# Algy/fast-slic

Measured on AMD Instinct MI355X. Metric: megapixels/sec @10 iters (1280x720 & 4K, K=1600); % HBM roofline, higher is better.
Workload: dtype u8/u16/i32 (integer SLIC); 1 GPU; 1280x720 RGB, K=1600, 10 iters (configs[1]), 8 frames/GPU; frames_per_gpu=8, global_frames=8, slots_per_gpu=6, submissions_per_launch_group=up to 2 (dynamic batching of the pipeline), inputs=device-resident uint8 RGB, device int16 labels, parallelism=frames sharded across GPUs, no collective

## Files before the change

### fast_slic_amd/csrc/cca.hip

```cpp
#include "device_common.h"

namespace fslic {

constexpr uint32_t kNoAdopt = 0xFFFFFFFFu;
static __device__ __forceinline__ uint32_t* n_parent(const CcaDev& c, uint32_t n) { return reinterpret_cast<uint32_t*>(c.nrec + n); }
static __device__ __forceinline__ uint32_t n_leader(const CcaDev& c, uint32_t n) { return reinterpret_cast<const uint32_t*>(c.nrec + n)[1]; }
static __device__ __forceinline__ uint32_t n_local(const CcaDev& c, uint32_t n) { return reinterpret_cast<const uint32_t*>(c.nrec + n)[2]; }
static __device__ __forceinline__ uint32_t n_adopt(const CcaDev& c, uint32_t n) { return reinterpret_cast<const uint32_t*>(c.nrec + n)[3]; }

static __device__ __forceinline__ uint32_t lds_ld(uint32_t* p) {
    return __hip_atomic_load(p, __ATOMIC_RELAXED, __HIP_MEMORY_SCOPE_WORKGROUP);
}
static __device__ __forceinline__ void lds_st(uint32_t* p, uint32_t v) {
    __hip_atomic_store(p, v, __ATOMIC_RELAXED, __HIP_MEMORY_SCOPE_WORKGROUP);
}
static __device__ __forceinline__ uint32_t lds_find(uint32_t* par, uint32_t x) {
    for (;;) {
        const uint32_t p = lds_ld(par + x);
        if (p == x) return x;
        const uint32_t gp = lds_ld(par + p);
        if (gp == p) return p;
        lds_st(par + x, gp);
        x = gp;
    }
// ... 261 lines not shown
static __device__ __forceinline__ uint32_t g_load(uint32_t* p) {
    return __hip_atomic_load(p, __ATOMIC_RELAXED, __HIP_MEMORY_SCOPE_AGENT);
}
static __device__ __forceinline__ uint32_t node_at(const CcaDev& c, int y, int x, size_t p) {
    return (uint32_t)((y / kCcaTileH) * c.tiles_x + x / kCcaTile) * (uint32_t)kCcaTilePx + (uint32_t)c.lid[p];
}
static __device__ __forceinline__ uint32_t node_of(const CcaDev& c, uint32_t p) {
    const int y = (int)(p / (uint32_t)c.W);
    return node_at(c, y, (int)(p - (uint32_t)y * (uint32_t)c.W), p);
}
static __device__ __forceinline__ uint32_t g_find(const CcaDev& c, uint32_t x) {
    for (;;) {
        const uint32_t p = g_load(n_parent(c, x));
        if (p == x) return x;
        const uint32_t gp = g_load(n_parent(c, p));
        if (gp == p) return p;
        __hip_atomic_store(n_parent(c, x), gp, __ATOMIC_RELAXED, __HIP_MEMORY_SCOPE_AGENT);
        x = gp;
    }
}
static __device__ __forceinline__ void g_union(const CcaDev& c, uint32_t a, uint32_t b) {
    for (;;) {
        a = g_find(c, a);
        b = g_find(c, b);
        if (a == b) return;
        if (n_leader(c, a) < n_leader(c, b)) { const uint32_t t = a; a = b; b = t; }
        if (atomicCAS(n_parent(c, a), a, b) == a) return;
    }
}

static __device__ __forceinline__ uint2 g_load2(const CcaDev& c, uint32_t n) {
    const unsigned long long v = __hip_atomic_load(reinterpret_cast<unsigned long long*>(c.nrec + n), __ATOMIC_RELAXED, __HIP_MEMORY_SCOPE_AGENT);
    return make_uint2((uint32_t)v, (uint32_t)(v >> 32));
}
static __device__ __forceinline__ uint32_t g_find_leader(const CcaDev& c, uint32_t& x, uint2 r) {
    for (;;) {
        if (r.x == x) return r.y;
        const uint2 g = g_load2(c, r.x);
        if (g.x == r.x) { x = r.x; return g.y; }
        __hip_atomic_store(n_parent(c, x), g.x, __ATOMIC_RELAXED, __HIP_MEMORY_SCOPE_AGENT);
        x = g.x;
        r = g_load2(c, x);
    }
}
static __device__ __forceinline__ void g_union2(const CcaDev& c, uint32_t a, uint32_t b) {
    uint2 ra = g_load2(c, a), rb = g_load2(c, b);
    for (;;) {
        const uint32_t la = g_find_leader(c, a, ra), lb = g_find_leader(c, b, rb);
        if (a == b) return;
        if (la < lb) { const uint32_t t = a; a = b; b = t; }
        if (atomicCAS(n_parent(c, a), a, b) == a) return;
        ra = g_load2(c, a); rb = g_load2(c, b);
    }
}

#ifndef FSLIC_SEAM_PX
#define FSLIC_SEAM_PX 1
#endif
constexpr int kSeamPx = FSLIC_SEAM_PX;
__global__ __launch_bounds__(256) void k_cca_border(CcaDev c, int nh, int nv) {
    c.select(blockIdx.y);
    constexpr int T = kCcaTile;
    constexpr int TH = kCcaTileH;
    static_assert(TH % kSeamPx == 0 && T % kSeamPx == 0, "a thread's pixels lie in one tile");
    const int i = blockIdx.x * blockDim.x + threadIdx.x;
    const int W = c.W, H = c.H;
    if (i < nh) {
        const int cw = (W + kSeamPx - 1) / kSeamPx;
        const int sr = i / cw, x0 = (i - sr * cw) * kSeamPx;
        const int y = (sr + 1) * TH;
        const size_t p = (size_t)y * W + x0;
        uint32_t cur[kSeamPx + 1], up[kSeamPx + 1], nc[kSeamPx], nu[kSeamPx];
        const bool has_left = (x0 % T) != 0;
        cur[0] = has_left ? (uint32_t)c.in[p - 1] : 0x10000u;
        up[0] = has_left ? (uint32_t)c.in[p - W - 1] : 0x10000u;
#pragma unroll
        for (int q = 0; q < kSeamPx; ++q) {
            const bool ok = x0 + q < W;
            cur[q + 1] = ok ? (uint32_t)c.in[p + q] : 0x20000u;
            up[q + 1] = ok ? (uint32_t)c.in[p - W + q] : 0x30000u;
            nc[q] = ok ? (uint32_t)c.lid[p + q] : 0u;
            nu[q] = ok ? (uint32_t)c.lid[p - W + q] : 0u;
        }
        const uint32_t tile = (uint32_t)((sr + 1) * c.tiles_x + x0 / T) * (uint32_t)kCcaTilePx;
#pragma unroll
        for (int q = 0; q < kSeamPx; ++q) {
            const uint32_t lbl = cur[q + 1];
            if (up[q + 1] == lbl && (cur[q] != lbl || up[q] != lbl))
                g_union2(c, tile + nc[q], tile - (uint32_t)c.tiles_x * (uint32_t)kCcaTilePx + nu[q]);
        }
    } else if (i < nh + nv) {
        const int j = i - nh;
        const int ch = (H + kSeamPx - 1) / kSeamPx;
        const int bx = j / ch + 1, y0 = (j - (bx - 1) * ch) * kSeamPx;
        const int r0 = y0 % TH;
        const uint32_t tile_r = (uint32_t)((y0 / TH) * c.tiles_x + bx), tile_l = tile_r - 1u;
        const uint32_t* er = c.vedge + ((size_t)tile_r * TH + r0) * 2;
        const uint32_t* el = c.vedge + ((size_t)tile_l * TH + r0) * 2 + 1;
        uint32_t a[kSeamPx + 1], b[kSeamPx + 1];
        a[0] = r0 ? er[-2] : 0x10000u;
        b[0] = r0 ? el[-2] : 0x20000u;
#pragma unroll
        for (int q = 0; q < kSeamPx; ++q) {
            const bool ok = y0 + q < H;
            a[q + 1] = ok ? er[2 * q] : 0x10000u;
            b[q + 1] = ok ? el[2 * q] : 0x20000u;
        }
#pragma unroll
        for (int q = 0; q < kSeamPx; ++q) {
            const uint32_t lbl = a[q + 1] & 0xFFFFu;
            const bool contact = y0 + q < H && ((a[q + 1] ^ b[q + 1]) & 0xFFFFu) == 0u;
            const bool first = q + r0 == 0 || (a[q] & 0xFFFFu) != lbl || (b[q] & 0xFFFFu) != lbl;
            if (contact && first)
                g_union2(c, tile_r * (uint32_t)kCcaTilePx + (a[q + 1] >> 16), tile_l * (uint32_t)kCcaTilePx + (b[q + 1] >> 16));
        }
    }
}

__global__ __launch_bounds__(256) void k_cca_compress(CcaDev c, int nframes) {
    const uint32_t bx = blockIdx.x / (unsigned)nframes, nbx = gridDim.x / (unsigned)nframes;
    c.select((int)(blockIdx.x % (unsigned)nframes));
    const uint32_t r_first = c.roots[bx * blockDim.x + threadIdx.x];
    const uint32_t n = c.counters[0];
    const int lane = LANE();
    const uint32_t gstride = nbx * blockDim.x;
    const int64_t thr = (int64_t)c.min_threshold;
    __shared__ uint32_t s_app[2];
    for (uint32_t b0 = bx * blockDim.x; b0 < n; b0 += gstride) {
        const uint32_t i = b0 + threadIdx.x;
        if (threadIdx.x == 0) s_app[0] = 0u;
        __syncthreads();
        const bool live = i < n;
        const uint32_t r = (b0 == bx * blockDim.x && live) ? r_first : c.roots[min(i, n - 1)];
        const uint32_t a = n_local(c, r);
        uint32_t g = r;
        for (;;) {
            const uint32_t p = g_load(n_parent(c, g));
            if (p == g) break;
            g = p;
        }
        bool cand = false;
        if (live) {
            if (g == r) {
                c.nfinal[r] = 0xFFFFu;
                cand = (int64_t)a >= thr;
            } else {
                __hip_atomic_store(n_parent(c, r), g, __ATOMIC_RELAXED, __HIP_MEMORY_SCOPE_AGENT);
                const uint32_t old = atomicAdd(&c.narea[g], a);
                cand = (int64_t)old < thr && (int64_t)old + (int64_t)a >= thr;
            }
        }
        const int32_t leader = cand ? (int32_t)n_leader(c, g) : 0;
        const unsigned long long m = __ballot(cand);
        uint32_t wbase = 0;
        if (m && lane == 0) wbase = atomicAdd(&s_app[0], (uint32_t)__popcll(m));
        wbase = rfl(wbase);
        __syncthreads();
        if (threadIdx.x == 0 && s_app[0]) s_app[1] = atomicAdd(&c.counters[1], s_app[0]);
        __syncthreads();
        if (cand) {
            const uint32_t at = s_app[1] + wbase + (uint32_t)__popcll(m & ((1ull << lane) - 1ull));
            c.cand_leader[at] = leader;
            c.cand_area[at] = g;
        }
    }
}

constexpr int kSelCap = 10240;
constexpr int kSelSortCap = 8192;
constexpr int kSelBuckets = 2048;
constexpr int kSelBins = 4096;

static __device__ __forceinline__ uint32_t block_excl_scan_1024(uint32_t v, uint32_t* s_w, uint32_t& total) {
    const int lane = threadIdx.x & 63, wave = threadIdx.x >> 6;
    uint32_t inc = v;
#pragma unroll
    for (int off = 1; off < 64; off <<= 1) {
        const uint32_t u = __shfl_up(inc, off);
        if (lane >= off) inc += u;
    }
    __syncthreads();
    if (lane == 63) s_w[wave] = inc;
    __syncthreads();
    uint32_t base = 0, tot = 0;
#pragma unroll
    for (int w = 0; w < 16; ++w) {
        const uint32_t t = s_w[w];
        if (w < wave) base += t;
        tot += t;
    }
    total = tot;
    return base + inc - v;
}

static __device__ __forceinline__ void select_pass(const uint32_t* s_area, uint32_t M, int sh, bool first, uint32_t prefix,
                                                   uint32_t kk, uint32_t* s_hist, uint32_t* s_w, uint32_t* s_v) {
    const int tid = threadIdx.x;
    for (int i = tid; i < kSelBins; i += 1024) s_hist[i] = 0;
    __syncthreads();
    for (uint32_t i = tid; i < M; i += 1024) {
        const uint32_t a = s_area[i];
        if (first || (a >> (sh + 12)) == prefix) atomicAdd(&s_hist[(a >> sh) & (kSelBins - 1)], 1u);
    }
    __syncthreads();
    uint32_t h[4], tot = 0;
#pragma unroll
    for (int q = 0; q < 4; ++q) { h[q] = s_hist[kSelBins - 1 - 4 * tid - q]; tot += h[q]; }
    uint32_t total;
    uint32_t run = block_excl_scan_1024(tot, s_w, total);
#pragma unroll
    for (int q = 0; q < 4; ++q) {
        if (run < kk && run + h[q] >= kk) {
            s_v[1] = (uint32_t)(kSelBins - 1 - 4 * tid - q);
            s_v[2] = kk - run;
        }
        run += h[q];
    }
    __syncthreads();
}

typedef unsigned long long heap_t;
constexpr int kTieWaveLevels = 4;
static __device__ __forceinline__ heap_t hp_ld(heap_t* p) { return __hip_atomic_load(p, __ATOMIC_RELAXED, __HIP_MEMORY_SCOPE_WORKGROUP); }
static __device__ __forceinline__ void hp_st(heap_t* p, heap_t v) { __hip_atomic_store(p, v, __ATOMIC_RELAXED, __HIP_MEMORY_SCOPE_WORKGROUP); }
static __device__ __forceinline__ uint32_t hp_area(heap_t e) { return (uint32_t)(e >> 32); }

static __device__ __forceinline__ void tie_adjust_heap(heap_t* h, int hole, int len, heap_t value, bool writer, uint32_t astar) {
    const uint32_t vlim = min(hp_area(value), astar);
    int cur = hole;
    for (;;) {
        int child;
        heap_t em;
        if (cur < (len - 1) / 2) {
            child = 2 * (cur + 1);
            const heap_t e1 = hp_ld(h + child), e0 = hp_ld(h + child - 1);
            em = e1;
            if (hp_area(e1) > hp_area(e0)) { child--; em = e0; }
        } else if ((len & 1) == 0 && cur == (len - 2) / 2) {
            child = 2 * cur + 1;
            em = hp_ld(h + child);
        } else {
            break;
        }
        if (hp_area(em) > vlim) break;
        if (writer) hp_st(h + cur, em);
        cur = child;
    }
    if (writer) hp_st(h + cur, value);
}

static __device__ __forceinline__ uint32_t tie_wave_sift(heap_t* h, int len, int hole, heap_t value, int lane, uint32_t astar) {
    constexpr uint32_t kInf = 0xFFFFFFFFu;
    const uint32_t va = hp_area(value);
    const uint32_t vlim = min(va, astar);
    const int t = 31 - __clz(lane | 1);
    const int off = lane - (1 << t);
    int cur = hole;
    uint32_t at_hole = va;
    for (;;) {
        const long long idx = (((long long)(cur + 1)) << t) + off - 1;
        const bool ok = lane >= 1 && idx < (long long)len;
        const heap_t e = ok ? hp_ld(h + idx) : ((heap_t)kInf << 32);
        const uint32_t a = (uint32_t)(e >> 32);
        const uint32_t sib = (uint32_t)__builtin_amdgcn_update_dpp(0, (int)a, 0xB1 , 0xF, 0xF, true);
        const unsigned long long left_pref = __ballot(sib > a);
        const unsigned long long stop_at = __ballot(a > vlim);
        int c[5];
        uint32_t stops = 0;
        {
            int jj = 1;
#pragma unroll
            for (int s5 = 0; s5 < 5; ++s5) {
                const int cl = 2 * jj;
                c[s5] = cl + (int)(((left_pref >> cl) & 1ull) ^ 1ull);
                stops |= (uint32_t)((stop_at >> c[s5]) & 1ull) << s5;
                jj = c[s5];
            }
        }
        const int nmove = __builtin_ctz(stops | 32u);
        const bool stopped = nmove < 5;
        unsigned long long path = 0;
        int j = 1;
#pragma unroll
        for (int s5 = 0; s5 < 5; ++s5) {
            path |= s5 < nmove ? 1ull << c[s5] : 0ull;
            j = s5 < nmove ? c[s5] : j;
        }
        const long long pidx = (((long long)(cur + 1)) << max(t - 1, 0)) + (off >> 1) - 1;
        if ((path >> lane) & 1ull) hp_st(h + pidx, e);
        if (cur == hole && (path & 0xCull)) at_hole = (uint32_t)__builtin_amdgcn_readlane((int)a, (path & 4ull) ? 2 : 3);
        const int tj = 31 - __clz(j);
        cur = (int)((((long long)(cur + 1)) << tj) + (j - (1 << tj)) - 1);
        if (stopped || 2 * cur + 1 >= len) break;
    }
    if (lane == 0) hp_st(h + cur, value);
    return at_hole;
}

#if defined(FSLIC_LAB) && FSLIC_LAB == 1
#define SEL_STAMP(i_) do { if (threadIdx.x == 0) c.counters[4 + (i_)] = (uint32_t)__builtin_amdgcn_s_memrealtime(); } while (0)
#else
#define SEL_STAMP(i_) do { } while (0)
#endif
static __device__ __forceinline__ void tie_heap_select(const CcaDev& c, uint32_t M, uint32_t K, uint32_t astar, uint32_t* s_area, uint32_t* s_lead, uint32_t* s_key,
                                                       uint32_t* s_bcnt, uint32_t* s_bstart, uint32_t* s_bfill, uint32_t* s_w) {
    const int tid = threadIdx.x, lane = tid & 63;
    SEL_STAMP(2);
    constexpr int PER = kSelSortCap / 1024;
    int bsh = 0;
    while ((((uint32_t)c.N - 1u) >> bsh) >= (uint32_t)kSelBuckets) bsh++;
    for (int i = tid; i < 3 * kSelBuckets; i += 1024) s_bcnt[i] = 0;
    __syncthreads();
    for (uint32_t i = tid; i < M; i += 1024) atomicAdd(&s_bcnt[s_lead[i] >> bsh], 1u);
    __syncthreads();
    {
        const uint32_t a = s_bcnt[2 * tid], b = s_bcnt[2 * tid + 1];
        uint32_t tot;
        const uint32_t ex = block_excl_scan_1024(a + b, s_w, tot);
        s_bstart[2 * tid] = ex;
        s_bstart[2 * tid + 1] = ex + a;
    }
    __syncthreads();
    for (uint32_t i = tid; i < M; i += 1024) {
        const uint32_t b = s_lead[i] >> bsh;
        s_key[s_bstart[b] + atomicAdd(&s_bfill[b], 1u)] = s_lead[i];
    }
    __syncthreads();
    uint32_t my_lead[PER], my_area[PER], my_rank[PER];
#pragma unroll
    for (int q = 0; q < PER; ++q) {
        const uint32_t i = (uint32_t)tid + (uint32_t)q * 1024u;
        my_lead[q] = 0; my_area[q] = 0; my_rank[q] = 0xFFFFFFFFu;
        if (i < M) {
            const uint32_t me = s_lead[i];
            const uint32_t b = me >> bsh;
            const uint32_t lo = s_bstart[b], hi = lo + s_bcnt[b];
            uint32_t r = lo;
            for (uint32_t j = lo; j < hi; ++j) r += (uint32_t)(s_key[j] < me);
            my_lead[q] = me; my_area[q] = s_area[i]; my_rank[q] = r;
        }
    }
    __syncthreads();
    heap_t* const heap = reinterpret_cast<heap_t*>(s_lead);
#pragma unroll
    for (int q = 0; q < PER; ++q)
        if (my_rank[q] != 0xFFFFFFFFu) {
            const uint32_t r = my_rank[q];
            c.cand_leader[r] = (int32_t)my_lead[q];
            s_area[r] = my_area[q];
            if (r < K) heap[r] = ((heap_t)my_area[q] << 32) | r;
        }
    uint32_t* const s_in = s_bcnt;
    static_assert(kSelSortCap / 32 <= 3 * kSelBuckets, "one bit per candidate in the bucket arrays");
    for (uint32_t w = (uint32_t)tid; w < (uint32_t)(kSelSortCap / 32); w += 1024u) {
        const uint32_t lo = w * 32u;
        s_in[w] = K >= lo + 32u ? 0xFFFFFFFFu : (K <= lo ? 0u : (1u << (K - lo)) - 1u);
    }
    __syncthreads();
    SEL_STAMP(3);
    const int len = (int)K;
    if (len >= 2) {
        const int last_parent = (len - 2) / 2;
        int d = 0;
        while (((2 << d) - 1) <= last_parent) d++;
        for (; d >= 0; --d) {
            const int lo = (1 << d) - 1, hi = min((2 << d) - 2, last_parent);
            if (d > kTieWaveLevels) {
                for (int p = lo + tid; p <= hi; p += 1024)
                    tie_adjust_heap(heap, p, len, hp_ld(heap + p), true, astar);
            } else {
                for (int p = lo + (int)rfl((uint32_t)(tid >> 6)); p <= hi; p += 16)
                    tie_wave_sift(heap, len, p, hp_ld(heap + p), lane, astar);
            }
            __syncthreads();
        }
    }
    SEL_STAMP(4);
    if (tid < 64) {
        constexpr uint32_t kInf = 0xFFFFFFFFu;
        uint32_t ea = kInf, ei = 0u;
        if (lane >= 1 && lane - 1 < len) { const heap_t e = hp_ld(heap + (lane - 1)); ea = hp_area(e); ei = (uint32_t)e; }
        uint32_t top_area = (uint32_t)__builtin_amdgcn_readlane((int)ea, 1);
        for (uint32_t base = K; base < M; base += 64) {
            const uint32_t i = base + (uint32_t)lane;
            const uint32_t a = i < M ? s_area[i] : 0u;
            unsigned long long m = __ballot(i < M && a > top_area);
            while (m) {
                const int j = __builtin_ctzll(m);
                m &= m - 1ull;
                const uint32_t aj = (uint32_t)__builtin_amdgcn_readlane((int)a, j);
                if (aj <= top_area) continue;
                const uint32_t vi = base + (uint32_t)j;
                const uint32_t ti = (uint32_t)__builtin_amdgcn_readlane((int)ei, 1);
                if (lane == 0) { atomicAnd(&s_in[ti >> 5], ~(1u << (ti & 31u))); atomicOr(&s_in[vi >> 5], 1u << (vi & 31u)); }
                const uint32_t vlim = min(aj, astar);
                const uint32_t sib = (uint32_t)__builtin_amdgcn_update_dpp(0, (int)ea, 0xB1 , 0xF, 0xF, true);
                const unsigned long long pref = (ballot(sib > ea) & 0x5555555555555554ull) | (ballot(sib >= ea) & 0xAAAAAAAAAAAAAAA8ull);
                const unsigned long long okm = (pref & ~ballot(ea > vlim)) | 3ull;
                uint32_t on = 1u;
#pragma unroll
                for (int s5 = 0; s5 < 5; ++s5) on &= (uint32_t)(okm >> (lane >> s5));
                const unsigned long long moved = ballot((on & 1u) != 0u) & ~3ull;
                const int dst = moved ? 63 - __builtin_clzll(moved) : 1;
                const uint32_t kids = lane < 32 ? (uint32_t)(moved >> (2 * lane)) & 3u : 0u;
                const int from = (kids ? 2 * lane + (int)(kids >> 1) : lane) << 2;
                ea = (uint32_t)__builtin_amdgcn_ds_bpermute(from, (int)ea);
                ei = (uint32_t)__builtin_amdgcn_ds_bpermute(from, (int)ei);
                const int cur = dst - 1;
                if (dst < 32 || 2 * cur + 1 >= len) {
                    if (lane == dst) { ea = aj; ei = vi; }
                } else {
                    (void)tie_wave_sift(heap, len, cur, ((heap_t)aj << 32) | (heap_t)vi, lane, astar);
                    const heap_t e = hp_ld(heap + cur);
                    if (lane == dst) { ea = hp_area(e); ei = (uint32_t)e; }
                }
                top_area = (uint32_t)__builtin_amdgcn_readlane((int)ea, 1);
            }
        }
    }
    __syncthreads();
    SEL_STAMP(5);
    uint32_t fl[PER], cnt = 0;
#pragma unroll
    for (int q = 0; q < PER; ++q) {
        const uint32_t i = (uint32_t)tid * PER + (uint32_t)q;
        fl[q] = i < M ? (uint32_t)(s_area[i] > astar) | ((s_in[i >> 5] >> (i & 31u)) & 1u) : 0u;
        cnt += fl[q];
    }
    uint32_t total;
    uint32_t run = block_excl_scan_1024(cnt, s_w, total);
    {
        uint32_t ld[PER], nd[PER];
#pragma unroll
        for (int q = 0; q < PER; ++q) ld[q] = (uint32_t)c.cand_leader[fl[q] ? (uint32_t)tid * PER + (uint32_t)q : 0u];
#pragma unroll
        for (int q = 0; q < PER; ++q) nd[q] = node_of(c, ld[q]);
#pragma unroll
        for (int q = 0; q < PER; ++q) {
            if (fl[q]) c.nfinal[nd[q]] = (uint16_t)run;
            run += fl[q];
        }
    }
    SEL_STAMP(6);
}

__global__ __launch_bounds__(1024) void k_cca_select(CcaDev c, int cap) {
    c.select(blockIdx.x);
    SEL_STAMP(0);
    extern __shared__ __attribute__((aligned(16))) uint32_t s_dyn[];
    uint32_t* const s_area = s_dyn;
    uint32_t* const s_lead = s_dyn + cap;
    uint32_t* const s_key = s_dyn + 2 * cap;
    uint32_t* const s_bcnt = s_dyn + 3 * cap;
    uint32_t* const s_bstart = s_bcnt + kSelBuckets;
    uint32_t* const s_bfill = s_bstart + kSelBuckets;
    uint32_t* const s_hist = s_bcnt;
    __shared__ uint32_t s_w[16];
    __shared__ uint32_t s_v[8];
    const int tid = threadIdx.x;
    const int lane = tid & 63;
    const int K = c.K;
    const uint32_t cand_last = (uint32_t)max(c.N, 2048) - 1u;
    uint32_t l_first[4], nd_first[4];
#pragma unroll
    for (int u = 0; u < 4; ++u) { l_first[u] = (uint32_t)c.cand_leader[min((uint32_t)threadIdx.x + 1024u * u, cand_last)]; nd_first[u] = c.cand_area[min((uint32_t)threadIdx.x + 1024u * u, cand_last)]; }
    const uint32_t M = c.counters[1];
    if (tid < 8) s_v[tid] = 0;
    if (tid == 0) c.counters[2] = M;
    if (M > (uint32_t)cap) {
        if (tid == 0) c.counters[3] = 2u;
        return;
    }
    uint32_t amax = 0;
    for (uint32_t i0 = tid; i0 < M; i0 += 4096) {
        uint32_t l[4], nd[4], a[4];
#pragma unroll
        for (int u = 0; u < 4; ++u) {
            if (i0 == (uint32_t)tid) { l[u] = l_first[u]; nd[u] = i0 + 1024u * u < M ? nd_first[u] : 0u; }
            else { l[u] = (uint32_t)c.cand_leader[min(i0 + 1024u * u, M - 1u)]; nd[u] = c.cand_area[min(i0 + 1024u * u, M - 1u)]; }
        }
#pragma unroll
        for (int u = 0; u < 4; ++u) a[u] = c.narea[nd[u]];
#pragma unroll
        for (int u = 0; u < 4; ++u) {
            const uint32_t i = i0 + 1024u * u;
            if (i < M) { s_area[i] = a[u]; s_lead[i] = l[u]; amax = max(amax, a[u]); }
        }
    }
    __syncthreads();
    if (M > (uint32_t)K) {
#pragma unroll
        for (int off = 32; off > 0; off >>= 1) amax = max(amax, (uint32_t)__shfl_xor(amax, off));
        if (lane == 0 && amax) atomicMax(&s_v[0], amax);
        __syncthreads();
    }
    uint32_t astar = 0;
    if (M > (uint32_t)K) {
        const uint32_t mx = s_v[0];
        int sh = 0;
        while ((mx >> sh) >= (uint32_t)kSelBins) sh += 12;
        uint32_t prefix = 0, kk = (uint32_t)K;
        bool first = true;
        for (; sh >= 0; sh -= 12) {
            select_pass(s_area, M, sh, first, prefix, kk, s_hist, s_w, s_v);
            prefix = (prefix << 12) | s_v[1];
            kk = s_v[2];
            first = false;
            __syncthreads();
        }
        astar = prefix;
        uint32_t eq = 0;
        for (uint32_t i = tid; i < M; i += 1024) eq += (uint32_t)(s_area[i] == astar);
#pragma unroll
        for (int off = 32; off > 0; off >>= 1) eq += (uint32_t)__shfl_xor(eq, off);
        if (lane == 0 && eq) atomicAdd(&s_v[4], eq);
        __syncthreads();
        SEL_STAMP(1);
        if (s_v[4] != kk) {
            if (M > (uint32_t)kSelSortCap) {
                if (tid == 0) c.counters[3] = 2u;
                return;
            }
            tie_heap_select(c, M, (uint32_t)K, astar, s_area, s_lead, s_key, s_bcnt, s_bstart, s_bfill, s_w);
            if (tid == 0) c.counters[3] = 0u;
            return;
        }
    }
    int bsh = 0;
    while ((((uint32_t)c.N - 1u) >> bsh) >= (uint32_t)kSelBuckets) bsh++;
    for (int i = tid; i < 3 * kSelBuckets; i += 1024) s_bcnt[i] = 0;
    __syncthreads();
    for (uint32_t i = tid; i < M; i += 1024)
        if (s_area[i] >= astar) atomicAdd(&s_bcnt[s_lead[i] >> bsh], 1u);
    __syncthreads();
    {
        const uint32_t a = s_bcnt[2 * tid], b = s_bcnt[2 * tid + 1];
        uint32_t n_keep;
        const uint32_t ex = block_excl_scan_1024(a + b, s_w, n_keep);
        s_bstart[2 * tid] = ex;
        s_bstart[2 * tid + 1] = ex + a;
    }
    __syncthreads();
    for (uint32_t i = tid; i < M; i += 1024)
        if (s_area[i] >= astar) {
            const uint32_t b = s_lead[i] >> bsh;
            s_key[s_bstart[b] + atomicAdd(&s_bfill[b], 1u)] = s_lead[i];
        }
    __syncthreads();
    for (uint32_t i0 = tid; i0 < M; i0 += 4096) {
        uint32_t me[4], r[4], nd[4];
        bool kept[4];
#pragma unroll
        for (int u = 0; u < 4; ++u) nd[u] = c.cand_area[min(i0 + 1024u * u, M - 1u)];
#pragma unroll
        for (int u = 0; u < 4; ++u) {
            const uint32_t i = i0 + 1024u * u;
            kept[u] = i < M && s_area[i] >= astar;
            me[u] = kept[u] ? s_lead[i] : 0u;
            r[u] = 0u;
            if (kept[u]) {
                const uint32_t b = me[u] >> bsh;
                const uint32_t lo = s_bstart[b], hi = lo + s_bcnt[b];
                r[u] = lo;
                for (uint32_t j = lo; j < hi; ++j) r[u] += (uint32_t)(s_key[j] < me[u]);
            }
        }
#pragma unroll
        for (int u = 0; u < 4; ++u) if (kept[u]) c.nfinal[nd[u]] = (uint16_t)r[u];
    }
    if (tid == 0) c.counters[3] = 0u;
}

static int root_pass_blocks(const CcaDev& c) {
    const int b = (c.N / 48 + 255) / 256;
    return b < 1 ? 1 : b;
}

void launch_cca_phase1(const CcaDev& c, int nframes, hipStream_t st) {
    constexpr int T = kCcaTile;
    const int tx = (c.W + T - 1) / T, ty = (c.H + kCcaTileH - 1) / kCcaTileH;
    launch(k_cca_local, dim3(nframes, tx, ty), dim3(256), 0, st, c);
    const int nh = (ty - 1) * ((c.W + kSeamPx - 1) / kSeamPx), nv = (tx - 1) * ((c.H + kSeamPx - 1) / kSeamPx);
    if (nh + nv > 0)
        launch(k_cca_border, dim3((nh + nv + 255) / 256, nframes), dim3(256), 0, st, c, nh, nv);
    launch(k_cca_compress, dim3(root_pass_blocks(c) * nframes), dim3(256), 0, st, c, nframes);
}

void launch_cca_select(const CcaDev& c, int nframes, hipStream_t st) {
    long long need = (long long)c.N / (c.min_threshold > 1 ? c.min_threshold : 1) + 1;
    int cap = 1024;
    while (cap < need && cap < kSelCap) cap <<= 1;
    if (cap > kSelCap) cap = kSelCap;
    const size_t lds = (3 * (size_t)cap + 3 * (size_t)kSelBuckets) * sizeof(uint32_t);
    static_assert(kSelBins <= 3 * kSelBuckets, "the selection histogram reuses the ranking buckets");
    static std::atomic<int> attr_state[64];
    if (!max_dynamic_lds_on_this_device(k_cca_select, (int)((3 * (size_t)kSelCap + 3 * (size_t)kSelBuckets) * sizeof(uint32_t)), attr_state)) {
        while (cap > 1024 && (3 * (size_t)cap + 3 * (size_t)kSelBuckets) * sizeof(uint32_t) > 64 * 1024) cap >>= 1;
        const size_t lds_small = (3 * (size_t)cap + 3 * (size_t)kSelBuckets) * sizeof(uint32_t);
        launch(k_cca_select, dim3(nframes), dim3(1024), lds_small, st, c, cap);
        return;
    }
    launch(k_cca_select, dim3(nframes), dim3(1024), lds, st, c, cap);
}

__global__ __launch_bounds__(256) void k_cca_reset_final(CcaDev c) {
    const uint32_t n = c.counters[0];
    for (uint32_t i = blockIdx.x * blockDim.x + threadIdx.x; i < n; i += gridDim.x * blockDim.x) {
        const uint32_t r = c.roots[i];
        if (*n_parent(c, r) == r) c.nfinal[r] = 0xFFFFu;
    }
}
__global__ void k_cca_set_kept(CcaDev c, const int32_t* __restrict__ leaders, const uint16_t* __restrict__ labels, int n) {
    const int i = blockIdx.x * blockDim.x + threadIdx.x;
    if (i < n) c.nfinal[node_of(c, (uint32_t)leaders[i])] = labels[i];
}
__global__ void k_cca_gather_area(CcaDev c) {
    const uint32_t M = c.counters[1];
    for (uint32_t i = blockIdx.x * blockDim.x + threadIdx.x; i < M; i += gridDim.x * blockDim.x) c.cand_area[i] = c.narea[node_of(c, (uint32_t)c.cand_leader[i])];
}
void launch_cca_gather_area(const CcaDev& c, hipStream_t st) {
    launch(k_cca_gather_area, dim3(64), dim3(256), 0, st, c);
}

void launch_cca_set_kept(const CcaDev& c, const int32_t* d_leaders, const uint16_t* d_labels, int n, hipStream_t st) {
    launch(k_cca_reset_final, dim3(root_pass_blocks(c)), dim3(256), 0, st, c);
    if (n <= 0) return;
    launch(k_cca_set_kept, dim3((n + 255) / 256), dim3(256), 0, st, c, d_leaders, d_labels, n);
}

static __device__ __forceinline__ uint32_t chase_final(const CcaDev& c, uint32_t g) {
    const uint32_t W = (uint32_t)c.W;
    for (;;) {
        const uint32_t cur = n_leader(c, g);
        if (cur == 0) return 0u;
        uint32_t a = n_adopt(c, g);
        if (a == kNoAdopt) {
            const uint32_t t = (cur % W > 0) ? cur - 1 : cur - W;
            a = node_of(c, t);
        }
        g = *n_parent(c, a);
        const uint32_t f = __hip_atomic_load(c.nfinal + g, __ATOMIC_RELAXED, __HIP_MEMORY_SCOPE_AGENT);
        if (f != 0xFFFFu) return f;
    }
}

__global__ __launch_bounds__(256) void k_cca_chain(CcaDev c) {
    c.select(blockIdx.y);
    const uint32_t i0 = blockIdx.x * blockDim.x + threadIdx.x;
    const uint32_t r0 = c.roots[i0];
    const uint32_t n = c.counters[0];
    const uint32_t gstride = gridDim.x * blockDim.x;
    for (uint32_t i = i0; i < n; i += gstride) {
        const uint32_t r = i == i0 ? r0 : c.roots[i];
        const uint32_t g = *n_parent(c, r);
        uint32_t f = __hip_atomic_load(c.nfinal + g, __ATOMIC_RELAXED, __HIP_MEMORY_SCOPE_AGENT);
        if (f == 0xFFFFu) f = chase_final(c, g);
        __hip_atomic_store(c.nfinal + r, (uint16_t)f, __ATOMIC_RELAXED, __HIP_MEMORY_SCOPE_AGENT);
    }
}

static __device__ __forceinline__ uint32_t wave_max_u32(uint32_t v) {
#define FSLIC_DPP_MAX(ctrl) v = max(v, (uint32_t)__builtin_amdgcn_update_dpp(0, (int)v, ctrl, 0xF, 0xF, false))
    FSLIC_DPP_MAX(0xB1); FSLIC_DPP_MAX(0x4E); FSLIC_DPP_MAX(0x141); FSLIC_DPP_MAX(0x140);
#undef FSLIC_DPP_MAX
    return max(max((uint32_t)__builtin_amdgcn_readlane((int)v, 0), (uint32_t)__builtin_amdgcn_readlane((int)v, 16)),
               max((uint32_t)__builtin_amdgcn_readlane((int)v, 32), (uint32_t)__builtin_amdgcn_readlane((int)v, 48)));
}

__global__ __launch_bounds__(256) void k_cca_relabel(CcaDev c, ExportDev ex, int relabel_blocks) {
    const int z = blockIdx.y;
    if ((int)blockIdx.x >= relabel_blocks) {
        const size_t d = (size_t)z * ex.frame_bytes;
        const uint32_t* yx = ex.yx_cur; const uint32_t* rest = ex.lab_n_moved; const uint32_t* misc = ex.misc0;
        FrameDev::adv(yx, d); FrameDev::adv(rest, d); FrameDev::adv(misc, d);
        uint32_t* out = ex.h_cl + (size_t)z * ex.h_stride;
        const int K = ex.K;
        for (int i = ((int)blockIdx.x - relabel_blocks) * blockDim.x + threadIdx.x; i < 4 * K; i += ((int)gridDim.x - relabel_blocks) * blockDim.x)
            out[i] = i < K ? yx[i] : rest[i - K];
        if ((int)blockIdx.x == relabel_blocks && threadIdx.x < 16) ex.h_misc[16 * (size_t)z + threadIdx.x] = misc[threadIdx.x];
        return;
    }
    c.select(z);
    constexpr int T = kCcaTile, TH = kCcaTileH;
    const int tiles_x = c.tiles_x, tiles_y = (c.H + TH - 1) / TH;
    const int ntiles = tiles_x * tiles_y;
    const bool vec = (c.W & 3) == 0;
    __shared__ __attribute__((aligned(16))) uint16_t s_fin[kCcaTilePx];
    __shared__ uint32_t s_max;
    for (int tile = blockIdx.x; tile < ntiles; tile += relabel_blocks) {
        const int ty = tile / tiles_x, tx = tile - ty * tiles_x;
        const uint16_t* __restrict__ gfin = c.nfinal + (size_t)tile * kCcaTilePx;
        const int x0 = tx * T + 4 * (int)(threadIdx.x & 15);
        const int r0 = (int)(threadIdx.x >> 4);
        if (tile != (int)blockIdx.x) __syncthreads();
        if (threadIdx.x == 0) s_max = 0u;
        __syncthreads();
        if (vec) {
            uint2 v[2];
            bool ok[2];
            uint32_t mx = 0;
#pragma unroll
            for (int h = 0; h < 2; ++h) {
                const int y = ty * TH + r0 + 16 * h;
                ok[h] = y < c.H && x0 < c.W;
                v[h] = make_uint2(0u, 0u);
                if (ok[h]) v[h] = *reinterpret_cast<const uint2*>(c.lid + (size_t)y * c.W + x0);
                mx = max(max(mx, max(v[h].x & 0xFFFFu, v[h].x >> 16)), max(v[h].y & 0xFFFFu, v[h].y >> 16));
            }
            mx = wave_max_u32(mx);
            if ((threadIdx.x & 63) == 0) atomicMax(&s_max, mx);
            __syncthreads();
            const uint32_t cnt = min(s_max + 1u, (uint32_t)kCcaTilePx);
            for (uint32_t i = threadIdx.x; i * 8u < cnt; i += 256u) reinterpret_cast<uint4*>(s_fin)[i] = reinterpret_cast<const uint4*>(gfin)[i];
            __syncthreads();
#pragma unroll
            for (int h = 0; h < 2; ++h) {
                if (!ok[h]) continue;
                const int y = ty * TH + r0 + 16 * h;
                uint2 o;
                o.x = (uint32_t)s_fin[v[h].x & 0xFFFFu] | ((uint32_t)s_fin[v[h].x >> 16] << 16);
                o.y = (uint32_t)s_fin[v[h].y & 0xFFFFu] | ((uint32_t)s_fin[v[h].y >> 16] << 16);
                st_stream(reinterpret_cast<uint2*>(c.out + (size_t)y * c.W + x0), o);
            }
        } else {
#pragma unroll
            for (int h = 0; h < 2; ++h) {
                const int y = ty * TH + r0 + 16 * h;
                if (y >= c.H) continue;
                for (int q = 0; q < 4; ++q) {
                    const int x = x0 + q;
                    if (x < c.W) st_stream(c.out + (size_t)y * c.W + x, gfin[c.lid[(size_t)y * c.W + x]]);
                }
            }
        }
    }
}

void launch_cca_phase2(const CcaDev& c, int nframes, hipStream_t st, const ExportDev* ex_) {
    launch(k_cca_chain, dim3(root_pass_blocks(c), nframes), dim3(256), 0, st, c);
    int blocks = c.tiles_x * ((c.H + kCcaTileH - 1) / kCcaTileH);
    const int cap = (16384 + nframes - 1) / nframes;
    if (blocks > cap) blocks = cap;
    if (blocks < 1) blocks = 1;
    ExportDev ex{};
    if (ex_) ex = *ex_;
    const int eb = ex.K > 0 ? (4 * ex.K + 1023) / 1024 : 0;
    launch(k_cca_relabel, dim3(blocks + eb, nframes), dim3(256), 0, st, c, ex, blocks);
}

}
```

### fast_slic_amd/csrc/clusters.hip

```cpp
#include "device_common.h"

namespace fslic {

template <int NB> struct EntryLoads { uint2 v[NB][3]; };
template <int NB> static __device__ __forceinline__ void request_entries(const FrameDev& f, int k, uint32_t e0, uint32_t ne, EntryLoads<NB>& L) {
    const char* cp = reinterpret_cast<const char*>(f.cpart + (size_t)k * f.cpart_ns * 6);
#pragma unroll
    for (int u = 0; u < NB; ++u) {
        const uint32_t e = min(e0 + (uint32_t)u, ne - 1u);
        const uint2* p = reinterpret_cast<const uint2*>(cp + __umul24(e, 24u));
        L.v[u][0] = p[0]; L.v[u][1] = p[1]; L.v[u][2] = p[2];
    }
}
static __device__ __forceinline__ bool entry_live(const FrameDev& f, const SlotGeom& g, uint32_t e, uint32_t ne, uint32_t ymask) {
    const uint32_t nbx = (uint32_t)f.nbx, xsh = 31u - (uint32_t)__clz((int)nbx);
    const uint32_t ry = ((e >> xsh) - (uint32_t)g.by0) & ymask, rx = (e - (uint32_t)g.bx0) & (nbx - 1u);
    return e < ne && ry <= (uint32_t)(g.by1 - g.by0) && rx <= (uint32_t)(g.bx1 - g.bx0);
}
template <int NB> static __device__ __forceinline__ void request_live_entries(const FrameDev& f, const SlotGeom& g, bool take, int k, uint32_t e0, uint32_t ne, uint32_t ymask, EntryLoads<NB>& L) {
    const char* cp = reinterpret_cast<const char*>(f.cpart + (size_t)k * f.cpart_ns * 6);
#pragma unroll
    for (int u = 0; u < NB; ++u) {
        const uint32_t e = e0 + (uint32_t)u;
        L.v[u][0] = L.v[u][1] = L.v[u][2] = make_uint2(0u, 0u);
        if (take && entry_live(f, g, e, ne, ymask)) {
            const uint2* p = reinterpret_cast<const uint2*>(cp + __umul24(e, 24u));
            L.v[u][0] = p[0]; L.v[u][1] = p[1]; L.v[u][2] = p[2];
        }
    }
}
template <int NB> static __device__ __forceinline__ void add_live_entries(const FrameDev& f, const SlotGeom& g, bool take, uint32_t e0, uint32_t ne, uint32_t ymask, const EntryLoads<NB>& L, uint32_t* out) {
#pragma unroll
    for (int u = 0; u < NB; ++u) {
        const bool livee = take && entry_live(f, g, e0 + (uint32_t)u, ne, ymask);
        out[0] += livee ? L.v[u][0].x : 0u; out[1] += livee ? L.v[u][0].y : 0u; out[2] += livee ? L.v[u][1].x : 0u;
        out[3] += livee ? L.v[u][1].y : 0u; out[4] += livee ? L.v[u][2].x : 0u; out[5] += livee ? L.v[u][2].y : 0u;
    }
}

template <int MODE, int NB>
static __device__ __forceinline__ void bin_clusters_body(FrameDev& f, const PassGeom& pg, const uint32_t* __restrict__ src_yx, size_t src_stride) {
    f.select(blockIdx.y);
    const uint32_t* __restrict__ yx_in = (MODE == 0 && src_yx) ? src_yx + (size_t)blockIdx.y * src_stride : f.cl_yx;
    const int gi = blockIdx.x * blockDim.x + threadIdx.x;
    if (gi < f.ncell) f.cell_cnt[1][gi] = 0;
    if (gi == 0) *f.ovf_cnt[1] = 0;
    const int k = MODE == 0 ? gi : (int)(blockIdx.x * (blockDim.x - 1) + threadIdx.x) - 1;
    const bool live = k >= 0 && k < f.K;
    uint32_t yx = live ? yx_in[k] : 0u;
    int y = (int)(yx >> 16), x = (int)(yx & 0xFFFF);
    uint32_t lab;
    bool shadowed = false;
    if (MODE == 0) {
        if (!live) return;
        lab = f.lab[(size_t)y * f.W + x] & 0x00FFFFFFu;
        f.cl_lab[k] = lab;
        f.cl_yx_out[k] = yx;
        if (src_yx) f.cl_yx[k] = yx;
        if (f.cl_f) {
            float* c = f.cl_f + 8 * (size_t)k;
            c[2] = (float)(lab & 255u); c[3] = (float)((lab >> 8) & 255u); c[4] = (float)((lab >> 16) & 255u);
        }
        shadowed = !f.cl_f && k > 0 && yx_in[k - 1] == yx;
        f.cl_shadow[k] = shadowed ? 1u : 0u;
    } else {
        const int kc = min(max(k, 0), f.K - 1);
        const uint32_t lab_own = f.cl_lab[kc];
        const uint32_t yx_prev = yx_in[max(kc - 1, 0)], lab_prev = f.cl_lab[max(kc - 1, 0)];
        const uint32_t shadow_word = f.cl_shadow[kc];
        const uint2* const sp = reinterpret_cast<const uint2*>(f.sums[0] + 6 * (size_t)kc);
        const uint2 s01 = sp[0], s23 = sp[1], s45 = sp[2];
        const uint32_t ymask = pg.use_slots ? cpart_rows_mask(f.S, pg.stride, max(pg.BH, 1)) : 0u, ne = pg.use_slots ? (ymask + 1u) * (uint32_t)f.nbx : 0u;
        EntryLoads<NB> L;
        if (NB == 4 && pg.use_slots) request_entries<NB>(f, kc, 0u, ne, L);
        const bool take = live && !(pg.use_slots && shadow_word);
        uint32_t s[6] = {0u, 0u, 0u, 0u, 0u, 0u};
        if (take) { s[0] = s01.x; s[1] = s01.y; s[2] = s23.x; s[3] = s23.y; s[4] = s45.x; s[5] = s45.y; }
        if (pg.use_slots) {
            const SlotGeom g = slot_geom((int)(yx >> 16), (int)(yx & 0xFFFFu), f.S, f.H, f.W, pg.rem, pg.stride, pg.BH, pg.Hv);
            if (NB == 4) {
                add_live_entries<NB>(f, g, take && g.any, 0u, ne, ymask, L, s);
            } else {
                for (uint32_t e0 = 0u; e0 < ne; e0 += (uint32_t)NB) {
                    request_live_entries<NB>(f, g, take && g.any, kc, e0, ne, ymask, L);
                    add_live_entries<NB>(f, g, take && g.any, e0, ne, ymask, L, s);
                }
            }
        }
        __shared__ uint32_t s_n[256];
        s_n[threadIdx.x] = s[0];
        __syncthreads();
        if (!live || threadIdx.x == 0) return;
        const uint32_t n_prev = s_n[threadIdx.x - 1];
        lab = lab_own;
        const uint32_t yx_prev_k = k > 0 ? yx_prev : 0u, lab_prev_k = k > 0 ? lab_prev : 0u;
        uint32_t* z0 = f.sums[1] + 6 * (size_t)k;
        const int32_t n = (int32_t)s[0];
        f.cl_n[k] = (uint32_t)n;
        if (n != 0) {
            const uint32_t h = (uint32_t)n >> 1, rcp = 0xFFFFFFFFu / (uint32_t)n;
            y = (int)div_by(s[1] + h, (uint32_t)n, rcp);
            x = (int)div_by(s[2] + h, (uint32_t)n, rcp);
            y = min(max(y, 0), f.H - 1);
            x = min(max(x, 0), f.W - 1);
            const int32_t L = (int32_t)div_by(s[3] + h, (uint32_t)n, rcp);
            const int32_t a = (int32_t)div_by(s[4] + h, (uint32_t)n, rcp);
            const int32_t b = (int32_t)div_by(s[5] + h, (uint32_t)n, rcp);
            if (f.cl_f) {
                float* c = f.cl_f + 8 * (size_t)k;
                const float fn = (float)n;
                const float fy = (float)(int32_t)s[1] / fn, fx = (float)(int32_t)s[2] / fn;
                c[0] = fy; c[1] = fx;
                c[2] = (float)(int32_t)s[3] / fn; c[3] = (float)(int32_t)s[4] / fn; c[4] = (float)(int32_t)s[5] / fn;
                y = min(max((int)fy, 0), f.H - 1);
                x = min(max((int)fx, 0), f.W - 1);
            }
            yx = ((uint32_t)y << 16) | (uint32_t)(x & 0xFFFF);
            lab = (uint32_t)(L & 255) | ((uint32_t)(a & 255) << 8) | ((uint32_t)(b & 255) << 16);
            f.cl_lab[k] = lab;
            f.cl_moved[k] = 1;
        } else if (!f.cl_f && k > 0 && n_prev == 0u) {
            shadowed = yx_prev_k == yx && lab_prev_k == lab;
        }
        f.cl_yx_out[k] = yx;
        f.cl_shadow[k] = shadowed ? 1u : 0u;
        z0[0] = 0; z0[1] = 0; z0[2] = 0; z0[3] = 0; z0[4] = 0; z0[5] = 0;
    }
    const uint32_t phase = 2u * (div_by((uint32_t)y, (uint32_t)f.T, f.T_rcp) & 1u) + (div_by((uint32_t)x, (uint32_t)f.T, f.T_rcp) & 1u);
    ClusterRec rec;
    rec.yx = yx; rec.lab = lab; rec.tag = (phase << 16) | (uint32_t)k; rec.pad = f.generation();
    f.cl_tag[k] = rec.tag;
    if (shadowed) return;
    const int cell = (y >> f.cs_shift) * f.ncx + (x >> f.cs_shift);
    const uint32_t slot = atomicAdd(&f.cell_cnt[0][cell], 1u);
    if (slot < (uint32_t)kCellCap) {
        f.cell_items[0][(size_t)cell * kCellCap + slot] = rec;
    } else {
        const uint32_t o = atomicAdd(f.ovf_cnt[0], 1u);
        f.ovf_items[0][o] = rec;
    }
}

template <int MODE, int NB = 8>
__global__ __launch_bounds__(256) void k_bin_clusters(FrameDev f, PassGeom pg, const uint32_t* __restrict__ src_yx, size_t src_stride) {
    bin_clusters_body<MODE, NB>(f, pg, src_yx, src_stride);
}

__global__ __launch_bounds__(256) void k_bin_clusters_lsc(FrameDev f, PassGeom pg, LscDev l, int nbin) {
    if ((int)blockIdx.x < nbin) {
        bin_clusters_body<1, 8>(f, pg, nullptr, (size_t)0);
        return;
    }
    l.select(blockIdx.y);
    const int t = ((int)blockIdx.x - nbin) * (int)blockDim.x + (int)threadIdx.x;
    const int k = t >> 4, q = t & 15;
    if (k >= f.K) return;
    long long* e = l.extra + (size_t)k * kLscExPitch;
    const long long mine = q <= kLscFeat ? e[q] : 0ll;
    const long long wsum = e[kLscFeat];
    const float acc = (float)((double)mine / (double)kLscFixF), tot_w = (float)((double)wsum / (double)kLscFixW);
    if (q < kLscFeat) l.cfeat[(size_t)k * kLscCfPitch + q] = acc / tot_w;
    __builtin_amdgcn_wave_barrier();
    if (q <= kLscFeat) e[q] = 0;
}

void launch_bin_clusters(const FrameDev& f_, int nframes, int mode, int buf, int sbuf, const PassGeom& pg, hipStream_t st,
                         const uint32_t* src_yx, size_t src_stride) {
    const FrameDev f = rotated(f_, buf, sbuf);
    if (mode == 0) {
        const int n = f.K > f.ncell ? f.K : f.ncell;
        launch((k_bin_clusters<0, 8>), dim3((n + 255) / 256, nframes), dim3(256), 0, st, f, pg, src_yx, src_stride);
    } else {
        const int bk = (f.K + 254) / 255, bc = (f.ncell + 255) / 256;
        int ne = 0;
        if (pg.use_slots) {
            const int n = (2 * f.S / pg.stride) / pg.BH + 2;
            int ny = 1;
            while (ny < n) ny <<= 1;
            ne = ny * f.nbx;
        }
        if (ne > 0 && ne <= 4) launch((k_bin_clusters<1, 4>), dim3(bk > bc ? bk : bc, nframes), dim3(256), 0, st, f, pg, nullptr, (size_t)0);
        else launch((k_bin_clusters<1, 8>), dim3(bk > bc ? bk : bc, nframes), dim3(256), 0, st, f, pg, nullptr, (size_t)0);
    }
}

void launch_bin_clusters_lsc(const FrameDev& f_, const LscDev& l, int nframes, int buf, int sbuf, hipStream_t st) {
    const FrameDev f = rotated(f_, buf, sbuf);
    const int bk = (f.K + 254) / 255, bc = (f.ncell + 255) / 256;
    const int nbin = bk > bc ? bk : bc;
    launch(k_bin_clusters_lsc, dim3(nbin + (f.K * 16 + 255) / 256, nframes), dim3(256), 0, st, f, PassGeom{}, l, nbin);
}

}
```

Baseline: 64860 megapixels/sec.

## Bin clusters with one block per frame using LDS cell counters; cache nodes in select

Adds a single-workgroup-per-frame cluster binning kernel. It walks all K clusters in 1024-thread chunks, prefetches the next chunk's loads, and keeps the per-cell counts in LDS atomics instead of global atomics. It carries the previous-cluster count across chunks and zeroes the other buffer's counters inside the same kernel. The tie-heap select also caches candidate node ids in LDS when they fit, which avoids a second global gather through cand_leader and node_of. The trade-off is much less parallelism per frame (one block), in exchange for fewer global atomics and less launch or memset work.

```diff
diff --git a/fast_slic_amd/csrc/cca.hip b/fast_slic_amd/csrc/cca.hip
--- a/fast_slic_amd/csrc/cca.hip
+++ b/fast_slic_amd/csrc/cca.hip
@@ -587,7 +587,7 @@
 #else
 #define SEL_STAMP(i_) do { } while (0)
 #endif
-static __device__ __forceinline__ void tie_heap_select(const CcaDev& c, uint32_t M, uint32_t K, uint32_t astar, uint32_t* s_area, uint32_t* s_lead, uint32_t* s_key,
+static __device__ __forceinline__ void tie_heap_select(const CcaDev& c, uint32_t M, uint32_t K, uint32_t astar, uint32_t cap, uint32_t* s_area, uint32_t* s_lead, uint32_t* s_key,
                                                        uint32_t* s_bcnt, uint32_t* s_bstart, uint32_t* s_bfill, uint32_t* s_w) {
     const int tid = threadIdx.x, lane = tid & 63;
     SEL_STAMP(2);
@@ -611,7 +611,11 @@
         s_key[s_bstart[b] + atomicAdd(&s_bfill[b], 1u)] = s_lead[i];
     }
     __syncthreads();
-    uint32_t my_lead[PER], my_area[PER], my_rank[PER];
+    const bool nodes_fit = 2u * K + M <= 2u * cap;
+    uint32_t* const s_node = s_lead + 2u * K;
+    uint32_t my_lead[PER], my_area[PER], my_rank[PER], my_node[PER];
+#pragma unroll
+    for (int q = 0; q < PER; ++q) my_node[q] = nodes_fit ? c.cand_area[min((uint32_t)tid + (uint32_t)q * 1024u, M - 1u)] : 0u;
 #pragma unroll
     for (int q = 0; q < PER; ++q) {
         const uint32_t i = (uint32_t)tid + (uint32_t)q * 1024u;
@@ -631,7 +635,8 @@
     for (int q = 0; q < PER; ++q)
         if (my_rank[q] != 0xFFFFFFFFu) {
             const uint32_t r = my_rank[q];
-            c.cand_leader[r] = (int32_t)my_lead[q];
+            if (nodes_fit) s_node[r] = my_node[q];
+            else c.cand_leader[r] = (int32_t)my_lead[q];
             s_area[r] = my_area[q];
             if (r < K) heap[r] = ((heap_t)my_area[q] << 32) | r;
         }
@@ -716,10 +721,15 @@
     uint32_t run = block_excl_scan_1024(cnt, s_w, total);
     {
         uint32_t ld[PER], nd[PER];
-#pragma unroll
-        for (int q = 0; q < PER; ++q) ld[q] = (uint32_t)c.cand_leader[fl[q] ? (uint32_t)tid * PER + (uint32_t)q : 0u];
-#pragma unroll
-        for (int q = 0; q < PER; ++q) nd[q] = node_of(c, ld[q]);
+        if (nodes_fit) {
+#pragma unroll
+            for (int q = 0; q < PER; ++q) nd[q] = fl[q] ? s_node[(uint32_t)tid * PER + (uint32_t)q] : 0u;
+        } else {
+#pragma unroll
+            for (int q = 0; q < PER; ++q) ld[q] = (uint32_t)c.cand_leader[fl[q] ? (uint32_t)tid * PER + (uint32_t)q : 0u];
+#pragma unroll
+            for (int q = 0; q < PER; ++q) nd[q] = node_of(c, ld[q]);
+        }
 #pragma unroll
         for (int q = 0; q < PER; ++q) {
             if (fl[q]) c.nfinal[nd[q]] = (uint16_t)run;
@@ -806,7 +816,7 @@
                 if (tid == 0) c.counters[3] = 2u;
                 return;
             }
-            tie_heap_select(c, M, (uint32_t)K, astar, s_area, s_lead, s_key, s_bcnt, s_bstart, s_bfill, s_w);
+            tie_heap_select(c, M, (uint32_t)K, astar, (uint32_t)cap, s_area, s_lead, s_key, s_bcnt, s_bstart, s_bfill, s_w);
             if (tid == 0) c.counters[3] = 0u;
             return;
         }
diff --git a/fast_slic_amd/csrc/clusters.hip b/fast_slic_amd/csrc/clusters.hip
--- a/fast_slic_amd/csrc/clusters.hip
+++ b/fast_slic_amd/csrc/clusters.hip
@@ -1,4 +1,8 @@
 #include "device_common.h"
+
+#ifndef FSLIC_BIN_BLOCK
+#define FSLIC_BIN_BLOCK 1024
+#endif
 
 namespace fslic {
 
@@ -36,6 +40,49 @@
         out[0] += livee ? L.v[u][0].x : 0u; out[1] += livee ? L.v[u][0].y : 0u; out[2] += livee ? L.v[u][1].x : 0u;
         out[3] += livee ? L.v[u][1].y : 0u; out[4] += livee ? L.v[u][2].x : 0u; out[5] += livee ? L.v[u][2].y : 0u;
     }
+}
+
+static __device__ __forceinline__ void update_cluster(const FrameDev& f, int k, const uint32_t* s, uint32_t lab_own, uint32_t yx_prev, uint32_t lab_prev, uint32_t n_prev,
+                                                      int& y, int& x, uint32_t& yx, uint32_t& lab, bool& shadowed) {
+    lab = lab_own;
+    const uint32_t yx_prev_k = k > 0 ? yx_prev : 0u, lab_prev_k = k > 0 ? lab_prev : 0u;
+    uint32_t* z0 = f.sums[1] + 6 * (size_t)k;
+    const int32_t n = (int32_t)s[0];
+    f.cl_n[k] = (uint32_t)n;
+    if (n != 0) {
+        const uint32_t h = (uint32_t)n >> 1, rcp = 0xFFFFFFFFu / (uint32_t)n;
+        y = (int)div_by(s[1] + h, (uint32_t)n, rcp);
+        x = (int)div_by(s[2] + h, (uint32_t)n, rcp);
+        y = min(max(y, 0), f.H - 1);
+        x = min(max(x, 0), f.W - 1);
+        const int32_t L = (int32_t)div_by(s[3] + h, (uint32_t)n, rcp);
+        const int32_t a = (int32_t)div_by(s[4] + h, (uint32_t)n, rcp);
+        const int32_t b = (int32_t)div_by(s[5] + h, (uint32_t)n, rcp);
+        if (f.cl_f) {
+            float* c = f.cl_f + 8 * (size_t)k;
+            const float fn = (float)n;
+            const float fy = (float)(int32_t)s[1] / fn, fx = (float)(int32_t)s[2] / fn;
+            c[0] = fy; c[1] = fx;
+            c[2] = (float)(int32_t)s[3] / fn; c[3] = (float)(int32_t)s[4] / fn; c[4] = (float)(int32_t)s[5] / fn;
+            y = min(max((int)fy, 0), f.H - 1);
+            x = min(max((int)fx, 0), f.W - 1);
+        }
+        yx = ((uint32_t)y << 16) | (uint32_t)(x & 0xFFFF);
+        lab = (uint32_t)(L & 255) | ((uint32_t)(a & 255) << 8) | ((uint32_t)(b & 255) << 16);
+        f.cl_lab[k] = lab;
+        f.cl_moved[k] = 1;
+    } else if (!f.cl_f && k > 0 && n_prev == 0u) {
+        shadowed = yx_prev_k == yx && lab_prev_k == lab;
+    }
+    f.cl_yx_out[k] = yx;
+    f.cl_shadow[k] = shadowed ? 1u : 0u;
+    z0[0] = 0; z0[1] = 0; z0[2] = 0; z0[3] = 0; z0[4] = 0; z0[5] = 0;
+}
+static __device__ __forceinline__ ClusterRec cluster_rec(const FrameDev& f, int k, int y, int x, uint32_t yx, uint32_t lab) {
+    const uint32_t phase = 2u * (div_by((uint32_t)y, (uint32_t)f.T, f.T_rcp) & 1u) + (div_by((uint32_t)x, (uint32_t)f.T, f.T_rcp) & 1u);
+    ClusterRec rec;
+    rec.yx = yx; rec.lab = lab; rec.tag = (phase << 16) | (uint32_t)k; rec.pad = f.generation();
+    return rec;
 }
 
 template <int MODE, int NB>
@@ -92,43 +139,9 @@
         __syncthreads();
         if (!live || threadIdx.x == 0) return;
         const uint32_t n_prev = s_n[threadIdx.x - 1];
-        lab = lab_own;
-        const uint32_t yx_prev_k = k > 0 ? yx_prev : 0u, lab_prev_k = k > 0 ? lab_prev : 0u;
-        uint32_t* z0 = f.sums[1] + 6 * (size_t)k;
-        const int32_t n = (int32_t)s[0];
-        f.cl_n[k] = (uint32_t)n;
-        if (n != 0) {
-            const uint32_t h = (uint32_t)n >> 1, rcp = 0xFFFFFFFFu / (uint32_t)n;
-            y = (int)div_by(s[1] + h, (uint32_t)n, rcp);
-            x = (int)div_by(s[2] + h, (uint32_t)n, rcp);
-            y = min(max(y, 0), f.H - 1);
-            x = min(max(x, 0), f.W - 1);
-            const int32_t L = (int32_t)div_by(s[3] + h, (uint32_t)n, rcp);
-            const int32_t a = (int32_t)div_by(s[4] + h, (uint32_t)n, rcp);
-            const int32_t b = (int32_t)div_by(s[5] + h, (uint32_t)n, rcp);
-            if (f.cl_f) {
-                float* c = f.cl_f + 8 * (size_t)k;
-                const float fn = (float)n;
-                const float fy = (float)(int32_t)s[1] / fn, fx = (float)(int32_t)s[2] / fn;
-                c[0] = fy; c[1] = fx;
-                c[2] = (float)(int32_t)s[3] / fn; c[3] = (float)(int32_t)s[4] / fn; c[4] = (float)(int32_t)s[5] / fn;
-                y = min(max((int)fy, 0), f.H - 1);
-                x = min(max((int)fx, 0), f.W - 1);
-            }
-            yx = ((uint32_t)y << 16) | (uint32_t)(x & 0xFFFF);
-            lab = (uint32_t)(L & 255) | ((uint32_t)(a & 255) << 8) | ((uint32_t)(b & 255) << 16);
-            f.cl_lab[k] = lab;
-            f.cl_moved[k] = 1;
-        } else if (!f.cl_f && k > 0 && n_prev == 0u) {
-            shadowed = yx_prev_k == yx && lab_prev_k == lab;
-        }
-        f.cl_yx_out[k] = yx;
-        f.cl_shadow[k] = shadowed ? 1u : 0u;
-        z0[0] = 0; z0[1] = 0; z0[2] = 0; z0[3] = 0; z0[4] = 0; z0[5] = 0;
-    }
-    const uint32_t phase = 2u * (div_by((uint32_t)y, (uint32_t)f.T, f.T_rcp) & 1u) + (div_by((uint32_t)x, (uint32_t)f.T, f.T_rcp) & 1u);
-    ClusterRec rec;
-    rec.yx = yx; rec.lab = lab; rec.tag = (phase << 16) | (uint32_t)k; rec.pad = f.generation();
+        update_cluster(f, k, s, lab_own, yx_prev, lab_prev, n_prev, y, x, yx, lab, shadowed);
+    }
+    const ClusterRec rec = cluster_rec(f, k, y, x, yx, lab);
     f.cl_tag[k] = rec.tag;
     if (shadowed) return;
     const int cell = (y >> f.cs_shift) * f.ncx + (x >> f.cs_shift);
@@ -144,6 +157,79 @@
 template <int MODE, int NB = 8>
 __global__ __launch_bounds__(256) void k_bin_clusters(FrameDev f, PassGeom pg, const uint32_t* __restrict__ src_yx, size_t src_stride) {
     bin_clusters_body<MODE, NB>(f, pg, src_yx, src_stride);
+}
+
+template <int NB> struct ClusterLoads {
+    uint32_t yx, lab_own, yx_prev, lab_prev, shadow_word;
+    uint2 s01, s23, s45;
+    EntryLoads<NB> L;
+};
+template <int NB> static __device__ __forceinline__ void request_cluster(const FrameDev& f, const PassGeom& pg, int kc, uint32_t ne, ClusterLoads<NB>& c) {
+    c.yx = f.cl_yx[kc];
+    c.lab_own = f.cl_lab[kc];
+    c.yx_prev = f.cl_yx[max(kc - 1, 0)]; c.lab_prev = f.cl_lab[max(kc - 1, 0)];
+    c.shadow_word = f.cl_shadow[kc];
+    const uint2* const sp = reinterpret_cast<const uint2*>(f.sums[0] + 6 * (size_t)kc);
+    c.s01 = sp[0]; c.s23 = sp[1]; c.s45 = sp[2];
+    if (NB == 4 && pg.use_slots) request_entries<NB>(f, kc, 0u, ne, c.L);
+}
+
+template <int NB, int BLOCK>
+__global__ __launch_bounds__(BLOCK) void k_bin_clusters_frame(FrameDev f, PassGeom pg) {
+    f.select(blockIdx.y);
+    extern __shared__ uint32_t s_cell[];
+    __shared__ uint32_t s_n[2][BLOCK + 1];
+    const int tid = threadIdx.x;
+    const uint32_t ymask = pg.use_slots ? cpart_rows_mask(f.S, pg.stride, max(pg.BH, 1)) : 0u, ne = pg.use_slots ? (ymask + 1u) * (uint32_t)f.nbx : 0u;
+    ClusterLoads<NB> cur;
+    request_cluster<NB>(f, pg, min(tid, f.K - 1), ne, cur);
+    for (int i = tid; i <= f.ncell; i += BLOCK) s_cell[i] = 0u;
+    for (int i = tid; i < f.ncell; i += BLOCK) f.cell_cnt[1][i] = 0;
+    if (tid == 0) *f.ovf_cnt[1] = 0;
+    for (int k0 = 0, par = 0; k0 < f.K; k0 += BLOCK, par ^= 1) {
+        const int k = k0 + tid;
+        const bool live = k < f.K;
+        ClusterLoads<NB> nxt;
+        if (k0 + BLOCK < f.K) request_cluster<NB>(f, pg, min(k + BLOCK, f.K - 1), ne, nxt);
+        uint32_t yx = cur.yx;
+        int y = (int)(yx >> 16), x = (int)(yx & 0xFFFF);
+        const bool take = live && !(pg.use_slots && cur.shadow_word);
+        uint32_t s[6] = {0u, 0u, 0u, 0u, 0u, 0u};
+        if (take) { s[0] = cur.s01.x; s[1] = cur.s01.y; s[2] = cur.s23.x; s[3] = cur.s23.y; s[4] = cur.s45.x; s[5] = cur.s45.y; }
+        if (pg.use_slots) {
+            const SlotGeom g = slot_geom(y, x, f.S, f.H, f.W, pg.rem, pg.stride, pg.BH, pg.Hv);
+            if (NB == 4) {
+                add_live_entries<NB>(f, g, take && g.any, 0u, ne, ymask, cur.L, s);
+            } else {
+                const int kc = min(k, f.K - 1);
+                for (uint32_t e0 = 0u; e0 < ne; e0 += (uint32_t)NB) {
+                    request_live_entries<NB>(f, g, take && g.any, kc, e0, ne, ymask, cur.L);
+                    add_live_entries<NB>(f, g, take && g.any, e0, ne, ymask, cur.L, s);
+                }
+            }
+        }
+        const uint32_t n_carry = s_n[par ^ 1][BLOCK];
+        s_n[par][tid + 1] = s[0];
+        __syncthreads();
+        if (live) {
+            const uint32_t n_prev = tid ? s_n[par][tid] : n_carry;
+            uint32_t lab;
+            bool shadowed = false;
+            update_cluster(f, k, s, cur.lab_own, cur.yx_prev, cur.lab_prev, n_prev, y, x, yx, lab, shadowed);
+            const ClusterRec rec = cluster_rec(f, k, y, x, yx, lab);
+            f.cl_tag[k] = rec.tag;
+            if (!shadowed) {
+                const int cell = (y >> f.cs_shift) * f.ncx + (x >> f.cs_shift);
+                const uint32_t slot = atomicAdd(&s_cell[cell], 1u);
+                if (slot < (uint32_t)kCellCap) f.cell_items[0][(size_t)cell * kCellCap + slot] = rec;
+                else f.ovf_items[0][atomicAdd(&s_cell[f.ncell], 1u)] = rec;
+            }
+        }
+        cur = nxt;
+    }
+    __syncthreads();
+    for (int i = tid; i < f.ncell; i += BLOCK) f.cell_cnt[0][i] = s_cell[i];
+    if (tid == 0) *f.ovf_cnt[0] = s_cell[f.ncell];
 }
 
 __global__ __launch_bounds__(256) void k_bin_clusters_lsc(FrameDev f, PassGeom pg, LscDev l, int nbin) {
@@ -179,6 +265,13 @@
             while (ny < n) ny <<= 1;
             ne = ny * f.nbx;
         }
+        constexpr int kFrameBinBlock = FSLIC_BIN_BLOCK, kFrameBinTrips = 6, kFrameBinCells = 4096;
+        if (f.K <= kFrameBinBlock * kFrameBinTrips && f.ncell <= kFrameBinCells) {
+            const size_t lds = ((size_t)f.ncell + 1) * sizeof(uint32_t);
+            if (ne > 0 && ne <= 4) launch((k_bin_clusters_frame<4, kFrameBinBlock>), dim3(1, nframes), dim3(kFrameBinBlock), lds, st, f, pg);
+            else launch((k_bin_clusters_frame<8, kFrameBinBlock>), dim3(1, nframes), dim3(kFrameBinBlock), lds, st, f, pg);
+            return;
+        }
         if (ne > 0 && ne <= 4) launch((k_bin_clusters<1, 4>), dim3(bk > bc ? bk : bc, nframes), dim3(256), 0, st, f, pg, nullptr, (size_t)0);
         else launch((k_bin_clusters<1, 8>), dim3(bk > bc ? bk : bc, nframes), dim3(256), 0, st, f, pg, nullptr, (size_t)0);
     }
```

After: 55670 megapixels/sec. 14.2% lower.
